# UMich-CURLY/SE3ET

Hardware: AMD Instinct MI355X
Metric: point-cloud pairs/sec (fwd), SE3ET-E 5k-pt pairs (higher is better)
Workload: dtype f32

## Files before the change

### include/se3et_hip.h

```cpp
#ifndef SE3ET_HIP_H_
#define SE3ET_HIP_H_

#include <stddef.h>
#include <stdint.h>

#ifdef __cplusplus
extern "C" {
#endif

#define SE3_OK 0
#define SE3_ERR_INVALID_ARG 1
#define SE3_ERR_UNSUPPORTED 2
#define SE3_ERR_LAUNCH 3
#define SE3_ERR_WORKSPACE 4

#define SE3_MAX_BATCH 32
#define SE3_MAX_NEIGHBOR_LIMIT 64

const char* se3_version(void);
const char* se3_last_error(void);
void se3_debug_set_sinkhorn_variant(int variant);
unsigned long long se3_debug_dense_saturated_rows(int reset);
unsigned long long se3_debug_attention_saturated(int reset);
void se3_debug_kernel_timing(int enable);
// ... 72 lines not shown
                         const float* residual_affine, float final_slope, int64_t rows, int channels,
                         const int64_t* segment_row_offsets_host, int num_segments, int blocked_layout, float* out, void* stream);
int se3_group_norm_apply_amax(const float* x, const float* affine_a, float slope_a, const float* affine_b, float slope_b, const float* residual,
                              const float* residual_affine, float final_slope, int64_t rows, int channels,
                              const int64_t* segment_row_offsets_host, int num_segments, int blocked_layout, float* out, float* amax_out,
                              void* stream);
size_t se3_dense_norm_workspace_bytes(int groups);
int se3_dense_norm_fwd(const float* x, int64_t rows, int in_features, const float* in_affine_a, float in_slope_a, const float* in_affine_b,
                       float in_slope_b, const void* weight_pieces, int out_features, const float* linear_bias, const float* norm_weight,
                       const float* norm_bias, int groups, float eps, const int64_t* segment_row_offsets_host, int num_segments, float* out,
                       float* affine_out, void* workspace, size_t workspace_bytes, void* stream);
int se3_dense_residual_fwd(const float* x, int64_t rows, int in_features, const float* in_affine_a, float in_slope_a, const float* in_affine_b,
                           float in_slope_b, const void* weight_pieces, const float* affine, const float* x2, int in_features2,
                           const void* weight_pieces2, const float* affine2, const float* residual, int out_features, float final_slope,
                           const int64_t* segment_row_offsets_host, int num_segments, float* out, void* stream);
int se3_linear_stream(const float* x, int64_t rows, int in_features, int64_t x_row_stride, const void* weight_pieces, const float* bias,
                      int out_features, int apply_relu, float* out, int64_t out_row_stride, void* stream);
int se3_linear_stream_transposed(const float* x, int64_t rows, int in_features, int64_t x_row_stride, const void* weight_pieces,
                                 const float* bias, int out_features, int block_rows, float* out_t, int64_t ld, void* stream);

int se3_add_layer_norm_fwd(const float* hidden, const float* hidden_bias, const float* residual, const float* weight,
                           const float* bias, int64_t rows, int64_t residual_rows, int channels, float eps, float* out,
                           void* stream);
int se3_add_layer_norm_bwd(const float* hidden, const float* hidden_bias, const float* residual, const float* weight,
                           const float* grad_out, int64_t rows, int64_t residual_rows, int channels, float eps, float* grad_hidden,
                           float* grad_params, void* stream);

size_t se3_linear_weight_pieces_bytes(int out_features, int in_features);
int se3_linear_split_weights_f16(const float* weight, int out_features, int in_features, void* pieces, void* stream);
int se3_linear_f16(const float* x, int64_t rows, int in_features, int64_t x_row_stride, const void* weight_pieces, const float* bias,
                   int out_features, int apply_relu, float* out, int64_t out_row_stride, void* stream);

int se3_gather_rows_padded(const float* x, const int64_t* idx, int64_t n, int64_t m, int64_t width, float* out,
                           void* stream);
int se3_neighbor_max_pool(const float* x, const int64_t* idx, int64_t n, int64_t m, int nn, int64_t width, float* out,
                          void* stream);
int se3_neighbor_max_pool_bwd(const float* x, const int64_t* idx, const float* dout, int64_t n, int64_t m, int nn, int64_t width,
                              float* dx, void* stream);
int se3_anchor_max(const float* x, int num_anchors, int64_t rows, int channels, int64_t anchor_stride, int64_t row_stride,
                   float* out, void* stream);

int se3_kpconv_so3_gather(const float* q_pts, const float* s_pts, const int64_t* idx, const float* x,
                          const float* kernel_points_host, const int64_t* kidx_host, const int64_t* ridx_host, float sigma,
                          int64_t num_queries, int64_t num_support, int num_neighbors, int in_channels, float* G,
                          void* stream);
int se3_kpconv_so3_gather_bwd(const float* q_pts, const float* s_pts, const int64_t* idx, const float* dG,
// ... 544 lines not shown
```

### se3et_amd/csrc/dense_norm.hip

```cpp
#include "common.h"
#include "group_norm.h"

namespace {

using f16x8 = __attribute__((ext_vector_type(8))) _Float16;
using f16x4 = __attribute__((ext_vector_type(4))) _Float16;
using f32x16 = __attribute__((ext_vector_type(16))) float;
using f32x4 = __attribute__((ext_vector_type(4))) float;
using u32x4 = __attribute__((ext_vector_type(4))) unsigned;
using i32x4 = __attribute__((ext_vector_type(4))) int;

__device__ unsigned long long g_dense_saturated_rows = 0;

template <int CTRL>
__device__ __forceinline__ float dpp_f32(float v) {
  return __builtin_bit_cast(float, __builtin_amdgcn_update_dpp(0, __builtin_bit_cast(int, v), CTRL, 0xf, 0xf, true));
}

constexpr int kHeaderB = 256;
constexpr int kRowB = 80;

struct DenseArgs {
  const float* x;
  const float* in_affine[2];
// ... 4 lines not shown
  float* out;
  float* part;
  int* counters;
  const float* xb;
  const float* gw;
  const float* gb;
  float* affine;
  int groups;
  float eps;
  SegTable T;
  const float* affine1;
  const float* residual;
  const float* x2;
  int K2;
  const u32x4* Wf2;
  const float* hdr2;
  const float* affine2;
  float final_slope;
  int x_rs, out_rs;
  int t_rows;
  int t_ld;
  int seg_steps;
  long long seg_stride;
};


struct StepPos {
  int tile, kk;
};
template <int WM, int WN, int RT, int CT, int MODE>
__global__ __launch_bounds__(256, MODE == 3 ? 2 : 3) void dense_norm_kernel(const DenseArgs a) {
  static_assert(WM * WN == 4, "4 waves");
  constexpr int TR = 32 * RT * WM, BN = 32 * CT * WN, U = TR / 32;
  constexpr int kPieceB = TR * kRowB, kBufB = 2 * kPieceB;
  constexpr bool kStats = MODE <= 1, kDual = MODE == 3, kPlain = MODE >= 4;
  __shared__ __align__(16) unsigned char lds[2 * kBufB];
  __shared__ __align__(16) int row_exp[2][TR];
  __shared__ __align__(16) int row_exp_step[2][TR];
  __shared__ int row_run[TR];
  __shared__ int row_scl[2];
  extern __shared__ __align__(16) float aff[];
  const int tid = threadIdx.x, lane = tid & 63, wave = __builtin_amdgcn_readfirstlane(tid >> 6);
  const int wm = wave / WN, wn = wave % WN;
  const int i32 = lane & 31, h = lane >> 5;
  const int K = a.K, N = a.N;
  const int K2 = kDual ? a.K2 : 32;
  const int XS = kPlain ? a.x_rs : K, OS = kPlain ? a.out_rs : N;
  long long r0, r1;
  chunk_rows(a.T, blockIdx.x, r0, r1);
  if (r1 < r0) r1 = r0;
  const int seg = seg_of_chunk(a.T, blockIdx.x);
  int cb0 = a.T.chunk_begin[0], cb1 = a.T.chunk_begin[1];
#pragma unroll
  for (int i = 1; i < kGNMaxSegments; i++)
// ... 151 lines not shown
    }
    const bool w_scaled = __builtin_amdgcn_ballot_w64(any_scaled) != 0;
    plain_rows = !w_scaled;
    if (last_step && w_scaled && lane == 0) row_scl[buf] = p.tile * nkt + p.kk;
    if (saturated) atomicAdd(&g_dense_saturated_rows, (unsigned long long)saturated);
  };
  const int a_read = (wm * (RT * 32) + i32) * kRowB + h * 16;
  const int ct0 = blockIdx.y * (BN / 32) + wn * CT;
  const u32x4* wbase1 = a.Wf + (int64_t)ct0 * 2 * 64 + lane;
  const u32x4* wbase2 = kDual ? a.Wf2 + (int64_t)ct0 * 2 * 64 + lane : wbase1;
  int coff[CT];
#pragma unroll
  for (int c = 0; c < CT; c++) coff[c] = kPlain ? ((ct0 + c < a.NCT ? ct0 + c : a.NCT - 1) - ct0) * 128 : c * 128;
  const int64_t wstep = (int64_t)a.NCT * 2 * 64;
  const float inv_scale = a.hdr[0];
  float fs[CT], bs[CT], rescale[CT];
#pragma unroll
  for (int c = 0; c < CT; c++) fs[c] = bs[c] = rescale[c] = 1.f;
  if constexpr (kPlain) {
#pragma unroll
    for (int c = 0; c < CT; c++) {
      const int col = (ct0 + c) * 32 + i32;
      fs[c] = inv_scale;
      bs[c] = (a.xb != nullptr && col < N) ? a.xb[col] : 0.f;
    }
  } else if constexpr (MODE >= 2) {
#pragma unroll
    for (int c = 0; c < CT; c++) {
      const int col = (ct0 + c) * 32 + i32;
      const float a1 = a.affine1[(size_t)seg * 2 * N + col], b1 = a.affine1[(size_t)seg * 2 * N + N + col];
      if constexpr (kDual) {
        const float a2 = a.affine2[(size_t)seg * 2 * N + col], b2 = a.affine2[(size_t)seg * 2 * N + N + col];
        const float inv2 = a.hdr2[0];
        rescale[c] = (a1 / a2) * (inv_scale / inv2);
        fs[c] = a2 * inv2;
        bs[c] = b1 + b2;
      } else {
        fs[c] = a1 * inv_scale;
        bs[c] = b1;
      }
    }
  }
  f32x16 acc[RT][CT];
#pragma unroll
  for (int r = 0; r < RT; r++)
#pragma unroll
    for (int c = 0; c < CT; c++)
// ... 107 lines not shown
    if constexpr (MODE == 5) {
      const __amdgpu_buffer_rsrc_t ors = __builtin_amdgcn_make_buffer_rsrc(a.out, 0, 0x7ffffff0, 0x00020000);
#pragma unroll
      for (int c = 0; c < CT; c++) {
        const int col = (ct0 + c) * 32 + i32;
#pragma unroll
        for (int r = 0; r < RT; r++)
#pragma unroll
          for (int g = 0; g < 4; g++) {
            const long long row = trow0 + r * 32 + 8 * g + 4 * h;
            const int blk = (int)(row / a.t_rows), rloc = (int)(row - (long long)blk * a.t_rows);
            f32x4 v4;
#pragma unroll
            for (int j = 0; j < 4; j++) {
              float val = acc[r][c][4 * g + j] * fs[c] + bs[c];
              v4[j] = fmaxf(val, val * a.final_slope);
              acc[r][c][4 * g + j] = 0.f;
            }
            const bool ok = col < N && row < r1;
            const int off = ok ? (int)((((long long)blk * N + col) * a.t_ld + rloc) * 4) : 0x7ffffff0;
            __builtin_amdgcn_raw_buffer_store_b128(__builtin_bit_cast(u32x4, v4), ors, off, 0, 0);
          }
      }
      return;
    }
    if constexpr (MODE >= 2) {
      const __amdgpu_buffer_rsrc_t ors = __builtin_amdgcn_make_buffer_rsrc(a.out + trow0 * N, 0, rows_here * N * 4, 0x00020000);
      const bool has_res = MODE == 2 && a.residual != nullptr;
      const __amdgpu_buffer_rsrc_t rrs = __builtin_amdgcn_make_buffer_rsrc(const_cast<float*>(has_res ? a.residual + trow0 * N : a.out), 0,
                                                                           has_res ? rows_here * N * 4 : 0, 0x00020000);
#pragma unroll
      for (int c = 0; c < CT; c++) {
        const int lane_off = (4 * h * N + (ct0 + c) * 32 + i32) * 4;
#pragma unroll
        for (int r = 0; r < RT; r++) {
          float res[16];
          if constexpr (MODE == 2) {
#pragma unroll
            for (int v = 0; v < 16; v++)
              res[v] = __builtin_bit_cast(float, __builtin_amdgcn_raw_buffer_load_b32(rrs, lane_off, (r * 32 + (v & 3) + 8 * (v >> 2)) * N * 4, 0));
          }
#pragma unroll
          for (int v = 0; v < 16; v++) {
            const int rr = r * 32 + (v & 3) + 8 * (v >> 2);
            float val = acc[r][c][v] * fs[c] + bs[c];
            if constexpr (MODE == 2) val += res[v];
// ... 95 lines not shown
#pragma unroll
    for (int c = 0; c < CT; c++) run[c].mean += a.xb[(ct0 + c) * 32 + i32];
  if (h == 0)
#pragma unroll
    for (int c = 0; c < CT; c++) sh[(wave * CT + c) * 32 + i32] = run[c];
  __syncthreads();
  if (wm == 0)
#pragma unroll
    for (int c = 0; c < CT; c++) {
      WF w = run[c];
      for (int m = 1; m < WM; m++) w = wf_merge(w, sh[((m * WN + wn) * CT + c) * 32 + i32]);
      for (int d = 1; d < cpg; d <<= 1) {
        const WF o = {__shfl_xor(w.n, d), __shfl_xor(w.mean, d), __shfl_xor(w.m2, d)};
        w = wf_merge(w, o);
      }
      const int col = (ct0 + c) * 32 + i32;
      if (h == 0 && (col & (cpg - 1)) == 0) gn_store_partial(a.part + ((int64_t)blockIdx.x * a.groups + col / cpg) * 3, w);
    }
  if (!gn_last_arrival(a.counters + seg * kGNMaxColumnBlocks + blockIdx.y, cb1 - cb0)) return;
  const int gpb = BN / cpg;
  gn_finalize_groups(a.part, a.groups, cb0, cb1, blockIdx.y * gpb, gpb, cpg, a.xb, a.gw, a.gb, a.eps, a.affine + (size_t)seg * 2 * N, N);
}

constexpr int kTargetChunks = 768;

}

extern "C" unsigned long long se3_debug_dense_saturated_rows(int reset) {
  unsigned long long n = 0;
  if (hipMemcpyFromSymbol(&n, HIP_SYMBOL(g_dense_saturated_rows), sizeof(n)) != hipSuccess) return ~0ull;
  if (reset) {
    const unsigned long long zero = 0;
    (void)hipMemcpyToSymbol(HIP_SYMBOL(g_dense_saturated_rows), &zero, sizeof(zero));
  }
  return n;
}

constexpr size_t kCounterB = kGNCounterB;

extern "C" size_t se3_dense_norm_workspace_bytes(int groups) {
  return kCounterB + (size_t)(kGNMaxChunks + kGNMaxSegments) * (groups > 0 ? groups : 1) * 3 * sizeof(float);
}

namespace {
int dense_chunks(int64_t rows, int N, const int64_t* segment_row_offsets_host, int num_segments, SegTable& T, int& TR, int& BN, int& ncb,
                 bool given = false) {
  if (!given) {
    TR = N >= 256 ? 64 : 128;
    BN = N >= 256 ? 256 : N;
  }
  ncb = (N + BN - 1) / BN;
  T = SegTable{};
  T.n = num_segments;
  T.quantum = TR;
  int64_t tiles = 0;
  for (int s = 0; s < num_segments; s++) {
    const int64_t b0 = num_segments == 1 ? 0 : segment_row_offsets_host[s], b1 = num_segments == 1 ? rows : segment_row_offsets_host[s + 1];
    if (!(b1 > b0 && b0 >= 0 && b1 <= rows)) return -1;
    tiles += se3_cdiv(b1 - b0, TR);
  }
  int64_t want = kTargetChunks / ncb;
  if (want > kGNMaxChunks - num_segments) want = kGNMaxChunks - num_segments;
  if (want < 1) want = 1;
  int64_t tiles_per_chunk = se3_cdiv(tiles, want);
  for (int s = 0; s < num_segments; s++) {
    const int64_t b0 = num_segments == 1 ? 0 : segment_row_offsets_host[s], b1 = num_segments == 1 ? rows : segment_row_offsets_host[s + 1];
    const int64_t need = se3_cdiv(se3_cdiv(b1 - b0, TR), 256);
    if (need > tiles_per_chunk) tiles_per_chunk = need;
  }
  int chunks = 0;
  for (int s = 0; s < num_segments; s++) {
    const int64_t b0 = num_segments == 1 ? 0 : segment_row_offsets_host[s], b1 = num_segments == 1 ? rows : segment_row_offsets_host[s + 1];
    T.row_begin[s] = b0;
    T.row_begin[s + 1] = b1;
    T.chunk_begin[s] = chunks;
    chunks += (int)se3_cdiv(se3_cdiv(b1 - b0, TR), tiles_per_chunk);
    T.chunk_begin[s + 1] = chunks;
  }
  if (!(T.row_begin[0] == 0 && T.row_begin[num_segments] == rows && chunks <= kGNMaxChunks + kGNMaxSegments)) return -1;
  return chunks;
}

template <int MODE>
void dense_launch(const DenseArgs& a, int N, dim3 grid, size_t dyn, hipStream_t st) {
// ... 99 lines not shown
  hipStream_t st = (hipStream_t)stream;
  const dim3 grid((unsigned)chunks, (unsigned)ncb);
  if (x2 != nullptr) {
    a.x2 = x2;
    a.K2 = K2;
    a.hdr2 = static_cast<const float*>(weight_pieces2);
    a.Wf2 = reinterpret_cast<const u32x4*>(static_cast<const unsigned char*>(weight_pieces2) + kHeaderB);
    a.affine2 = affine2;
    dense_launch<3>(a, N, grid, dyn, st);
  } else {
    dense_launch<2>(a, N, grid, dyn, st);
  }
  SE3_CHECK_LAUNCH("dense_residual");
  return SE3_OK;
}


namespace {
template <int WM, int WN, int RT, int CT>
void plain_launch(const DenseArgs& a, bool transposed, dim3 grid, hipStream_t st) {
  if (transposed) dense_norm_kernel<WM, WN, RT, CT, 5><<<grid, 256, 0, st>>>(a);
  else dense_norm_kernel<WM, WN, RT, CT, 4><<<grid, 256, 0, st>>>(a);
}
int linear_stream_one(const float* x, int64_t rows, int K, int64_t x_rs, const void* weight_pieces, const float* bias, int N, int relu, float* out,
                      int64_t out_rs, int t_rows, int64_t t_ld, void* stream, int seg_channels = 0, int64_t seg_stride = 0) {
  SE3_REQUIRE(x && weight_pieces && out, SE3_ERR_INVALID_ARG, "linear_stream: null pointer");
  SE3_REQUIRE(K > 0 && K % 32 == 0 && N > 0, SE3_ERR_UNSUPPORTED, "linear_stream: in_features %d must be a multiple of 32", K);
  SE3_REQUIRE(x_rs >= 4 && x_rs % 4 == 0 && ((uintptr_t)x & 15) == 0 && rows * x_rs < (1ll << 29), SE3_ERR_INVALID_ARG,
              "linear_stream: x rows must be 16-byte aligned, row stride %lld, below 2 GB", (long long)x_rs);
  const bool transposed = t_rows > 0;
  if (transposed)
    SE3_REQUIRE(t_rows % 4 == 0 && rows % t_rows == 0 && t_ld >= t_rows && t_ld % 4 == 0 && ((uintptr_t)out & 15) == 0 &&
                    (rows / t_rows) * N * t_ld < (1ll << 29),
                SE3_ERR_INVALID_ARG, "linear_stream: transposed output blocks of %d rows (a multiple of 4 dividing %lld), leading dimension %lld",
                t_rows, (long long)rows, (long long)t_ld);
  else
    SE3_REQUIRE(out_rs >= N && rows * out_rs < (1ll << 29), SE3_ERR_INVALID_ARG, "linear_stream: out row stride %lld", (long long)out_rs);
  if (rows == 0) return SE3_OK;
  int TR, BN, cfg;
  const int64_t rt64 = se3_cdiv(rows, 64);
  if (N > 128) {
    if (rt64 * se3_cdiv(N, 256) >= 512) { TR = 64; BN = 256; cfg = 0; }
    else if (rt64 * se3_cdiv(N, 128) >= 320 || N % 128 > 64) { TR = 64; BN = 128; cfg = 1; }
    else { TR = 64; BN = 64; cfg = 2; }
  } else if (N > 64) { TR = rt64 >= 512 ? 128 : 64; BN = 128; cfg = rt64 >= 512 ? 3 : 1; }
  else if (N > 32) { TR = rt64 >= 512 ? 128 : 64; BN = 64; cfg = rt64 >= 512 ? 4 : 2; }
  else { TR = 128; BN = 32; cfg = 5; }
  if (transposed && cfg == 3) { TR = 64; cfg = 1; }
  SegTable T;
  int ncb;
  const int chunks = dense_chunks(rows, N, nullptr, 1, T, TR, BN, ncb, true);
  SE3_REQUIRE(chunks > 0, SE3_ERR_INVALID_ARG, "linear_stream: %lld rows", (long long)rows);
  DenseArgs a{};
  a.x = x;
  a.K = K;
  a.N = N;
  a.NCT = (N + 63) / 64 * 2;
  a.hdr = static_cast<const float*>(weight_pieces);
  a.Wf = reinterpret_cast<const u32x4*>(static_cast<const unsigned char*>(weight_pieces) + kHeaderB);
  a.out = out;
  a.xb = bias;
  a.T = T;
  a.final_slope = relu ? 0.f : 1.f;
  a.x_rs = (int)x_rs;
  a.out_rs = (int)out_rs;
  a.t_rows = t_rows;
  a.t_ld = (int)t_ld;
  if (seg_channels > 0) {
    SE3_REQUIRE(seg_channels % 32 == 0 && K % seg_channels == 0 && seg_stride >= rows * x_rs && (K / seg_channels) * seg_stride < (1ll << 29),
                SE3_ERR_INVALID_ARG, "linear_stream: %d input channels in segments of %d", K, seg_channels);
    a.seg_steps = seg_channels / 32;
    a.seg_stride = seg_stride;
  }
  hipStream_t st = (hipStream_t)stream;
  const dim3 grid((unsigned)chunks, (unsigned)ncb);
  switch (cfg) {
    case 0: plain_launch<1, 4, 2, 2>(a, transposed, grid, st); break;
    case 1: plain_launch<2, 2, 1, 2>(a, transposed, grid, st); break;
    case 2: plain_launch<2, 2, 1, 1>(a, transposed, grid, st); break;
    case 3: plain_launch<2, 2, 2, 2>(a, transposed, grid, st); break;
    case 4: plain_launch<4, 1, 1, 2>(a, transposed, grid, st); break;
    default: plain_launch<4, 1, 1, 1>(a, transposed, grid, st); break;
  }
  SE3_CHECK_LAUNCH("linear_stream");
  return SE3_OK;
}

int linear_stream(const float* x, int64_t rows, int K, int64_t x_rs, const void* weight_pieces, const float* bias, int N, int relu, float* out,
                  int64_t out_rs, int t_rows, int64_t t_ld, void* stream, int seg_channels = 0, int64_t seg_stride = 0) {
  const int64_t lim = (1ll << 29) - 1;
  const bool transposed = t_rows > 0;
  const bool fits = rows >= 0 && x_rs > 0 && rows * x_rs <= lim &&
                    (transposed ? (rows / t_rows) * (int64_t)N * t_ld <= lim : rows * (out_rs > N ? out_rs : (int64_t)N) <= lim);
  if (fits || seg_channels > 0 || !x || !out || N <= 0) return linear_stream_one(x, rows, K, x_rs, weight_pieces, bias, N, relu, out, out_rs, t_rows, t_ld, stream, seg_channels, seg_stride);
  int64_t step;
  if (transposed) {
    SE3_REQUIRE(rows % t_rows == 0 && t_ld >= t_rows, SE3_ERR_INVALID_ARG, "linear_stream: transposed output blocks of %d rows", t_rows);
    const int64_t per_block = std::max((int64_t)t_rows * x_rs, (int64_t)N * t_ld);
    SE3_REQUIRE(per_block <= lim, SE3_ERR_UNSUPPORTED, "linear_stream: one transposed block of %d rows exceeds 2 GB", t_rows);
    step = lim / per_block * t_rows;
  } else {
    SE3_REQUIRE(out_rs >= N, SE3_ERR_INVALID_ARG, "linear_stream: out row stride %lld", (long long)out_rs);
    step = lim / std::max(x_rs, out_rs) / 256 * 256;
    SE3_REQUIRE(step > 0, SE3_ERR_UNSUPPORTED, "linear_stream: row strides %lld / %lld too large", (long long)x_rs, (long long)out_rs);
  }
  for (int64_t r0 = 0; r0 < rows; r0 += step) {
    const int64_t n = std::min(step, rows - r0);
    float* o = transposed ? out + (r0 / t_rows) * (int64_t)N * t_ld : out + r0 * out_rs;
    const int rc = linear_stream_one(x + r0 * x_rs, n, K, x_rs, weight_pieces, bias, N, relu, o, out_rs, t_rows, t_ld, stream);
    if (rc != SE3_OK) return rc;
  }
  return SE3_OK;
}
}

extern "C" int se3_linear_stream(const float* x, int64_t rows, int in_features, int64_t x_row_stride, const void* weight_pieces, const float* bias,
                                 int out_features, int apply_relu, float* out, int64_t out_row_stride, void* stream) {
  return linear_stream(x, rows, in_features, x_row_stride, weight_pieces, bias, out_features, apply_relu, out, out_row_stride, 0, 0, stream);
}

extern "C" int se3_linear_stream_transposed(const float* x, int64_t rows, int in_features, int64_t x_row_stride, const void* weight_pieces,
                                            const float* bias, int out_features, int block_rows, float* out_t, int64_t ld, void* stream) {
  SE3_REQUIRE(block_rows > 0, SE3_ERR_INVALID_ARG, "linear_stream_transposed: block_rows %d", block_rows);
  return linear_stream(x, rows, in_features, x_row_stride, weight_pieces, bias, out_features, 0, out_t, 0, block_rows, ld, stream);
}


extern "C" int se3_linear_stream_segments(const float* x, int64_t rows, int in_features, int seg_channels, int64_t seg_stride,
                                          const void* weight_pieces, const float* bias, int out_features, int apply_relu, float* out,
                                          int64_t out_row_stride, void* stream) {
  SE3_REQUIRE(seg_channels > 0, SE3_ERR_INVALID_ARG, "linear_stream_segments: seg_channels %d", seg_channels);
  return linear_stream(x, rows, in_features, seg_channels, weight_pieces, bias, out_features, apply_relu, out, out_row_stride, 0, 0, stream,
                       seg_channels, seg_stride);
}
```

### se3et_amd/csrc/transformer_driver.hip

```cpp
#include <cstddef>
#include <hip/hip_runtime.h>

#include <cmath>
#include <cstring>

#include "../../include/se3et_hip.h"
#include "common.h"

namespace {

struct Arena {
  unsigned char* base;
  size_t size, used;
  bool ok;
  void* take(size_t bytes) {
    const size_t at = se3_align256(used);
    if (at + bytes > size) {
      ok = false;
      return base;
    }
    used = at + bytes;
    return base + at;
  }
  float* floats(size_t n) { return static_cast<float*>(take(n * sizeof(float))); }
};

struct Half {
  int64_t row0, rows;
  int64_t starts[SE3_MAX_BATCH], lengths[SE3_MAX_BATCH];
  int n;
};

#define SE3_TRY(call)          \
  do {                         \
    const int rc_ = (call);    \
    if (rc_ != SE3_OK) return rc_; \
  } while (0)

int dense(const se3_linear_t& L, const float* x, int64_t rows, float* out, int relu, bool with_bias, void* st) {
  return se3_linear_stream(x, rows, L.in_features, L.in_features, L.pieces, with_bias ? L.bias : nullptr, L.out_features, relu, out,
                           L.out_features, st);
}

int ffn(const se3_layer_t& L, const float* y, int64_t rows, int C, float* out, Arena& S, void* st) {
  float* mid = S.floats((size_t)rows * L.expand.out_features);
  float* sq = S.floats((size_t)rows * C);
  if (!S.ok) return SE3_ERR_WORKSPACE;
  SE3_TRY(dense(L.expand, y, rows, mid, 1, true, st));
  SE3_TRY(dense(L.squeeze, mid, rows, sq, 0, false, st));
  return se3_add_layer_norm_fwd(sq, L.squeeze.bias, y, L.ln2_w, L.ln2_b, rows, rows, C, L.ln2_eps, out, st);
}

int copy_rows(float* dst, int64_t dst_pitch_floats, const float* src, int64_t src_pitch_floats, int64_t width_floats, int64_t height, hipStream_t st) {
  if (hipMemcpy2DAsync(dst, (size_t)dst_pitch_floats * 4, src, (size_t)src_pitch_floats * 4, (size_t)width_floats * 4, (size_t)height,
                       hipMemcpyDeviceToDevice, st) != hipSuccess) {
    se3_set_error("transformer_forward: device copy failed");
    return SE3_ERR_LAUNCH;
  }
  return SE3_OK;
}

int zero(float* p, size_t n, hipStream_t st) {
  if (hipMemsetAsync(p, 0, n * sizeof(float), st) != hipSuccess) {
    se3_set_error("transformer_forward: memset failed");
    return SE3_ERR_LAUNCH;
  }
  return SE3_OK;
}

int eq_groups(int A, const Half& q, int H, int C, const Half& k, int64_t v_row_stride) {
  if (C / H != 64 || C % H || A > 6 || v_row_stride % 16) return 1;
  for (int i = 0; i < k.n; i++)
    if (k.starts[i] % 16) return 1;
// ... 85 lines not shown
      float* vt = W.floats((size_t)As * C * R);
      float* hidden = W.floats((size_t)rows * C);
      size_t lg = 0;
      for (int c = 0; c < 2 * B; c++) lg += (size_t)As * H * plan->lengths[c] * ((plan->lengths[c] + 31) / 32 * 32);
      float* logits = W.floats(lg);
      const size_t kvb = se3_attention_kv_pieces_bytes(As, R, C, (int)R);
      void* kv = kvb ? W.take(kvb) : nullptr;
      float* lin = W.floats((size_t)rows * C);
      float* y = W.floats((size_t)rows * C);
      if (!W.ok) { se3_set_error("transformer_forward: workspace exhausted (self block %d)", bi); return SE3_ERR_WORKSPACE; }
      SE3_TRY(dense(L.stack, src, rows, proj, 0, true, stream));
      SE3_TRY(se3_linear_stream_transposed(src, rows, C, C, L.v.pieces, L.v.bias, C, (int)R, vt, R, stream));
      SE3_TRY(zero(hidden, (size_t)rows * C, st));
      const float* const* eqp = eq ? plan->eq : nullptr;
      const float* qe = eq ? proj + L.off_qe : nullptr;
      if (plan->emb_bf16)
        SE3_TRY(se3_rpe_self_attention_stack_bf16_fwd(proj + L.off_q, proj + L.off_k, vt, proj + L.off_qp, qe, NS, As > 1 ? (int64_t)R * NS : 0, (int)R,
                                                      As > 1 ? (int64_t)C * R : 0, reinterpret_cast<const uint16_t* const*>(plan->emb), eqp, plan->starts,
                                                      plan->lengths, 2 * B, As, C, H, logits, As > 1 ? (int64_t)R * C : 0, hidden, kv, kvb, stream));
      else
        SE3_TRY(se3_rpe_self_attention_stack_fwd(proj + L.off_q, proj + L.off_k, vt, proj + L.off_qp, qe, NS, As > 1 ? (int64_t)R * NS : 0, (int)R,
                                                 As > 1 ? (int64_t)C * R : 0, plan->emb, eqp, plan->starts, plan->lengths, 2 * B, As, C, H, logits,
                                                 As > 1 ? (int64_t)R * C : 0, hidden, kv, kvb, stream));
      SE3_TRY(dense(L.out, hidden, rows, lin, 0, false, stream));
      SE3_TRY(se3_add_layer_norm_fwd(lin, L.out.bias, src, L.ln1_w, L.ln1_b, rows, rows, C, L.ln1_eps, y, stream));
      float* Xn = free_slot(X, Xeq);
      SE3_TRY(ffn(L, y, rows, C, Xn, W, stream));
      if (L.type == 1 && next == 2) {
        float* inv = free_slot(Xn, X, Xeq);
        SE3_TRY(se3_anchor_max(Xn, A, R, C, (int64_t)R * C, C, inv, stream));
        Xeq = Xn;
        X = inv;
        X_is_eq = false;
      } else {
        X = Xn;
        X_is_eq = As > 1;
      }
    } else if (L.type == 2) {
      SE3_REQUIRE(!X_is_eq, SE3_ERR_UNSUPPORTED, "transformer_forward: block %d: plain cross attention on anchor features", bi);
      const bool eq_values = next == 1 || (next < 0 && prev == 1);
      SE3_REQUIRE(!eq_values || Xeq != nullptr, SE3_ERR_INVALID_ARG, "transformer_forward: block %d needs the anchor features of a self_eq block", bi);
      const int Av = eq_values ? A : 1;
      float* Xn = free_slot(X, Xeq);
      float* Xeqn = eq_values ? free_slot(X, Xeq, Xn) : nullptr;
      auto direction = [&](const Half& Pq, const Half& Pk, const float* xq, const float* xk, const float* xv, int64_t xv_pitch, float* y_out ) -> int {
        const int64_t Rq = Pq.rows, Rk = Pk.rows;
        float* q = W.floats((size_t)Rq * C);
        float* k = W.floats((size_t)Rk * C);
        float* xvc = W.floats((size_t)Av * Rk * C);
        float* vt = W.floats((size_t)Av * C * Rk);
        float* hidden = W.floats((size_t)Av * Rq * C);
        float* lin = W.floats((size_t)Av * Rq * C);
        float* y = W.floats((size_t)Av * Rq * C);
        if (!W.ok) { se3_set_error("transformer_forward: workspace exhausted (cross block %d)", bi); return SE3_ERR_WORKSPACE; }
        SE3_TRY(dense(L.q, xq, Rq, q, 0, true, stream));
        SE3_TRY(dense(L.k, xk, Rk, k, 0, true, stream));
        const float* xvv = xv;
        if (Av > 1 && xv_pitch != Rk * C) {
          SE3_TRY(copy_rows(xvc, Rk * C, xv, xv_pitch, Rk * C, Av, st));
          xvv = xvc;
        }
        SE3_TRY(se3_linear_stream_transposed(xvv, (int64_t)Av * Rk, C, C, L.v.pieces, L.v.bias, C, (int)Rk, vt, Rk, stream));
        SE3_TRY(zero(hidden, (size_t)Av * Rq * C, st));
        SE3_TRY(se3_attention_stack_fwd(q, k, vt, nullptr, Pq.starts, Pq.lengths, Pk.starts, Pk.lengths, nullptr, Pq.n, Av, C, H, C, C, (int)Rk, 0, 0,
                                        Av > 1 ? (int64_t)C * Rk : 0, Av > 1 ? (int64_t)Rq * C : 0, scale, hidden, nullptr, 0, stream));
        SE3_TRY(dense(L.out, hidden, (int64_t)Av * Rq, lin, 0, false, stream));
        SE3_TRY(se3_add_layer_norm_fwd(lin, L.out.bias, xq, L.ln1_w, L.ln1_b, (int64_t)Av * Rq, Rq, C, L.ln1_eps, y, stream));
        return ffn(L, y, (int64_t)Av * Rq, C, y_out, W, stream);
      };
      if (eq_values) {
        float* y0 = W.floats((size_t)A * R0 * C);
        float* y1 = W.floats((size_t)A * R1 * C);
        SE3_TRY(direction(P0, P1, X, X + R0 * C, Xeq + R0 * C, (int64_t)R * C, y0));
        SE3_TRY(se3_anchor_max(y0, A, R0, C, (int64_t)R0 * C, C, Xn, stream));
        SE3_TRY(direction(P1, P0, X + R0 * C, Xn, y0, (int64_t)R0 * C, y1));
        SE3_TRY(se3_anchor_max(y1, A, R1, C, (int64_t)R1 * C, C, Xn + R0 * C, stream));
        SE3_TRY(copy_rows(Xeqn, R * C, y0, R0 * C, R0 * C, A, st));
        SE3_TRY(copy_rows(Xeqn + R0 * C, R * C, y1, R1 * C, R1 * C, A, st));
        Xeq = Xeqn;
      } else {
        SE3_TRY(direction(P0, P1, X, X + R0 * C, X + R0 * C, 0, Xn));
        SE3_TRY(direction(P1, P0, X + R0 * C, Xn, Xn, 0, Xn + R0 * C));
      }
      X = Xn;
      X_is_eq = false;
    } else {
      SE3_REQUIRE(X_is_eq && A == 6, SE3_ERR_UNSUPPORTED, "transformer_forward: block %d: equivariant cross attention needs (6, rows, C) features", bi);
      const int mode = L.type == 3 ? 0 : 1;
      float* y0 = W.floats((size_t)A * R0 * C);
      float* y1 = W.floats((size_t)A * R1 * C);
// ... 8 lines not shown
        float* hidden = W.floats((size_t)A * Rq * G * C);
        float* gq = W.floats((size_t)A * B * C * C);
        float* gk = W.floats((size_t)A * B * C * C);
        float* partial = W.floats((size_t)B * A * A);
        float* weights = W.floats((size_t)B * (mode == 0 ? A * A : L.num_rotations));
        const size_t x6b = se3_cross_eq_x6_workspace_bytes(A, Rq, Rk, C, (int)Rk);
        void* x6 = W.take(x6b);
        float* lin = W.floats((size_t)A * Rq * C);
        float* y = W.floats((size_t)A * Rq * C);
        if (!W.ok) { se3_set_error("transformer_forward: workspace exhausted (equivariant cross block %d)", bi); return SE3_ERR_WORKSPACE; }
        SE3_TRY(dense(L.q, xq, (int64_t)A * Rq, q, 0, true, stream));
        SE3_TRY(dense(L.k, xk, (int64_t)A * Rk, k, 0, true, stream));
        SE3_TRY(se3_linear_stream_transposed(xk, (int64_t)A * Rk, C, C, L.v.pieces, L.v.bias, C, (int)Rk, vt, Rk, stream));
        SE3_TRY(zero(hidden, (size_t)A * Rq * G * C, st));
        SE3_TRY(se3_gram_stack(q, A, C, (int64_t)Rq * C, Pq.starts, Pq.lengths, B, gq, stream));
        SE3_TRY(se3_gram_stack(k, A, C, (int64_t)Rk * C, Pk.starts, Pk.lengths, B, gk, stream));
        const float f = 1.0f / (std::sqrt((float)(C / H)) * (float)H);
        SE3_TRY(se3_gram_frobenius(gq, gk, A, B, (int64_t)C * C, f * f, partial, stream));
        SE3_TRY(se3_cross_eq_stack_x6_fwd(q, k, vt, Pq.starts, Pq.lengths, Pk.starts, Pk.lengths, B, A, C, H, Rq, Rk, (int64_t)Rq * C, (int64_t)Rk * C,
                                          (int)Rk, (int64_t)C * Rk, mode, L.trace_idx, L.num_rotations, 1, partial, mix, weights, hidden, G,
                                          (int64_t)Rq * G * C, x6, x6b, stream));
        const void* wp = G == 1 ? L.out.pieces : (G == 2 ? L.out_pieces_g2 : L.out_pieces_g3);
        SE3_REQUIRE(wp != nullptr, SE3_ERR_INVALID_ARG, "transformer_forward: block %d: no output projection for %d key-anchor groups", bi, G);
        SE3_TRY(se3_linear_stream(hidden, (int64_t)A * Rq, G * C, (int64_t)G * C, wp, nullptr, C, 0, lin, C, stream));
        SE3_TRY(se3_add_layer_norm_fwd(lin, L.out.bias, xq, L.ln1_w, L.ln1_b, (int64_t)A * Rq, (int64_t)A * Rq, C, L.ln1_eps, y, stream));
        return ffn(L, y, (int64_t)A * Rq, C, y_out, W, stream);
      };
      float* xq0 = W.floats((size_t)A * R0 * C);
      float* xk0 = W.floats((size_t)A * R1 * C);
      if (!W.ok) { se3_set_error("transformer_forward: workspace exhausted (equivariant cross block %d)", bi); return SE3_ERR_WORKSPACE; }
      SE3_TRY(copy_rows(xq0, R0 * C, X, R * C, R0 * C, A, st));
      SE3_TRY(copy_rows(xk0, R1 * C, X + R0 * C, R * C, R1 * C, A, st));
      SE3_TRY(direction(P0, P1, xq0, xk0, mix0, y0));
      SE3_TRY(direction(P1, P0, xk0, y0, mix1, y1));
      float* Xn = free_slot(X, Xeq);
      if (L.type == 4 && next >= 0 && next != 1 && next < 3) {
        SE3_REQUIRE(plan->rc_expand.pieces && plan->rc_squeeze.pieces, SE3_ERR_INVALID_ARG, "transformer_forward: block %d needs the rotcompress layer", bi);
        float* y1p = W.floats((size_t)A * R1 * C);
        SE3_TRY(se3_anchor_mix_stack(y1, R1, C, mix0, P1.starts, P1.lengths, B, y1p, stream));
        auto rotcompress = [&](const float* x, int64_t Rh, float* o) -> int {
          float* mx = W.floats((size_t)Rh * C);
          float* mid = W.floats((size_t)Rh * plan->rc_expand.out_features);
          float* sq = W.floats((size_t)Rh * C);
          if (!W.ok) { se3_set_error("transformer_forward: workspace exhausted (rotcompress)"); return SE3_ERR_WORKSPACE; }
          SE3_TRY(se3_anchor_max(x, A, Rh, C, Rh * C, C, mx, stream));
          SE3_TRY(se3_linear_stream_segments(x, Rh, A * C, C, Rh * C, plan->rc_expand.pieces, plan->rc_expand.bias, plan->rc_expand.out_features, 1, mid,
                                             plan->rc_expand.out_features, stream));
          SE3_TRY(dense(plan->rc_squeeze, mid, Rh, sq, 0, false, stream));
          return se3_add_layer_norm_fwd(sq, plan->rc_squeeze.bias, mx, plan->rc_ln_w, plan->rc_ln_b, Rh, Rh, C, plan->rc_ln_eps, o, stream);
        };
        SE3_TRY(rotcompress(y0, R0, Xn));
        SE3_TRY(rotcompress(y1p, R1, Xn + R0 * C));
        X = Xn;
        X_is_eq = false;
        Xeq = nullptr;
      } else {
        SE3_TRY(copy_rows(Xn, R * C, y0, R0 * C, R0 * C, A, st));
        SE3_TRY(copy_rows(Xn + R0 * C, R * C, y1, R1 * C, R1 * C, A, st));
        X = Xn;
        X_is_eq = true;
      }
    }
  }
  SE3_REQUIRE(!X_is_eq, SE3_ERR_UNSUPPORTED, "transformer_forward: the block list must end on invariant features");
  return dense(plan->out_proj, X, R, out, 0, true, stream);
}
```

### se3et_amd/ops.py

```python
import ctypes
import os
import threading

import torch

from .caches import CACHE_EPOCH, Derived, Workspace, _Shared, also_clear, clear_caches, clear_weight_caches, validate_weight_caches
from ._lib import CONSTANTS, ENUMS, check, lib
from .stacking import PAIR_MAX_PAIRS, device_offsets, exclusive_offsets, to_device


_HAS_BLAS_SWITCH = hasattr(torch.backends.cuda, 'preferred_blas_library')
if _HAS_BLAS_SWITCH:
    torch.backends.cuda.preferred_blas_library('cublas')
_BLAS_SWITCH_LOCK = threading.Lock()
_BIG_GEMM_FLOP = 2.0e9


def mm(a, b):
    big = 2.0 * a.shape[0] * a.shape[1] * b.shape[1] > _BIG_GEMM_FLOP
    if _HAS_BLAS_SWITCH and big and (b.stride(-1) == 1 or a.shape[1] <= 32):
        with _BLAS_SWITCH_LOCK:
            torch.backends.cuda.preferred_blas_library('cublaslt')
            try:
                return torch.mm(a, b)
# ... 85 lines not shown
    if out is None:
        out = torch.empty(x.shape[:-1] + (N,), dtype=torch.float32, device=x.device)
        out_rs = N
    else:
        if out.dim() != 2 or out.shape[0] != rows or out.shape[1] != N or out.stride(1) != 1 or out.dtype != torch.float32:
            raise RuntimeError('linear_stream: out must be a (rows, N) float32 view with unit column stride')
        out_rs = out.stride(0)
    b = None if bias is None else _req(bias.detach().contiguous(), torch.float32, 'bias', 1)
    check(lib().se3_linear_stream(x.data_ptr(), rows, K, x_rs, Wp.data_ptr(), None if b is None else b.data_ptr(), N, 1 if relu else 0,
                                  out.data_ptr(), out_rs, stream), 'se3_linear_stream')
    return out


def linear_stream_transposed(x, weight, bias, ld=None):
    A, R, K = x.shape
    N = weight.shape[0]
    ld = R if ld is None else int(ld)
    stream = _stream()
    Wp = _linear_weight_pieces(weight, stream)
    out = torch.empty((A, N, ld), dtype=torch.float32, device=x.device)
    b = None if bias is None else _req(bias.detach().contiguous(), torch.float32, 'bias', 1)
    check(lib().se3_linear_stream_transposed(x.data_ptr(), A * R, K, K, Wp.data_ptr(), None if b is None else b.data_ptr(), N, R, out.data_ptr(), ld,
                                             stream), 'se3_linear_stream_transposed')
    return out


TIMING_TAG = None
KERNEL_TIMINGS = None
_TIMING_LOCK = threading.Lock()


class _timed:
    def __init__(self, name, nbytes, kind=None):
        self.name, self.nbytes, self.kind = name, nbytes, kind

    def __enter__(self):
        if KERNEL_TIMINGS is not None:
            self.e0, self.e1 = torch.cuda.Event(enable_timing=True), torch.cuda.Event(enable_timing=True)
            self.e0.record()

    def __exit__(self, *exc):
        if KERNEL_TIMINGS is not None:
            self.e1.record()
            KERNEL_TIMINGS.setdefault(self.name, []).append((self.e0, self.e1, self.nbytes))
            if self.kind is not None:
                KERNEL_TIMINGS.setdefault(self.name + '/' + self.kind, []).append((self.e0, self.e1, self.nbytes))
# ... 2477 lines not shown
```

Baseline: 465.5.

## Fuse output projection with residual add and LayerNorm in linear stream kernel

Adds a new epilogue mode to the dense GEMM kernel that adds bias and residual, computes per-row mean and variance through a cross-wave LDS reduction, and writes LayerNorm output directly. The transformer driver's attention-output, FFN-squeeze and rotation-compress projections now use this fused path instead of a GEMM followed by a separate add-layernorm launch. This removes one kernel launch and a full write/read round-trip of the intermediate per call. In exchange, each block must cover the full row width (128 or 256 columns), which constrains tiling and occupancy and adds two block syncs.

Measured after the change: 461.1. No clear change (-0.9%).

```diff
diff --git a/include/se3et_hip.h b/include/se3et_hip.h
--- a/include/se3et_hip.h
+++ b/include/se3et_hip.h
@@ -118,6 +118,9 @@
 int se3_add_layer_norm_fwd(const float* hidden, const float* hidden_bias, const float* residual, const float* weight,
                            const float* bias, int64_t rows, int64_t residual_rows, int channels, float eps, float* out,
                            void* stream);
+int se3_linear_layer_norm_stream(const float* x, int64_t rows, int in_features, int64_t x_row_stride, const void* weight_pieces,
+                                 const float* linear_bias, int out_features, const float* residual, int64_t residual_rows,
+                                 const float* ln_weight, const float* ln_bias, float eps, float* out, float* scratch, void* stream);
 int se3_add_layer_norm_bwd(const float* hidden, const float* hidden_bias, const float* residual, const float* weight,
                            const float* grad_out, int64_t rows, int64_t residual_rows, int channels, float eps, float* grad_hidden,
                            float* grad_params, void* stream);
diff --git a/se3et_amd/csrc/dense_norm.hip b/se3et_amd/csrc/dense_norm.hip
--- a/se3et_amd/csrc/dense_norm.hip
+++ b/se3et_amd/csrc/dense_norm.hip
@@ -50,6 +50,12 @@
   int t_ld;
   int seg_steps;
   long long seg_stride;
+  const float* ln_w;
+  const float* ln_b;
+  float ln_eps;
+  int res_rows;
+  int res_row0;
+  int res_bytes;
 };
 
 
@@ -57,7 +63,7 @@
   int tile, kk;
 };
 template <int WM, int WN, int RT, int CT, int MODE>
-__global__ __launch_bounds__(256, MODE == 3 ? 2 : 3) void dense_norm_kernel(const DenseArgs a) {
+__global__ __launch_bounds__(256, (MODE == 3 || (MODE == 6 && (RT == 2 || WM == 2))) ? 2 : 3) void dense_norm_kernel(const DenseArgs a) {
   static_assert(WM * WN == 4, "4 waves");
   constexpr int TR = 32 * RT * WM, BN = 32 * CT * WN, U = TR / 32;
   constexpr int kPieceB = TR * kRowB, kBufB = 2 * kPieceB;
@@ -255,7 +261,7 @@
     for (int c = 0; c < CT; c++) {
       const int col = (ct0 + c) * 32 + i32;
       fs[c] = inv_scale;
-      bs[c] = (a.xb != nullptr && col < N) ? a.xb[col] : 0.f;
+      bs[c] = (MODE != 6 && a.xb != nullptr && col < N) ? a.xb[col] : 0.f;
     }
   } else if constexpr (MODE >= 2) {
 #pragma unroll
@@ -409,6 +415,127 @@
             __builtin_amdgcn_raw_buffer_store_b128(__builtin_bit_cast(u32x4, v4), ors, off, 0, 0);
           }
       }
+      return;
+    }
+    if constexpr (MODE == 6) {
+#pragma clang fp contract(off)
+      int tid_here = tid;
+      asm volatile("" : "+v"(tid_here));
+      const int lane = tid_here & 63, i32 = lane & 31, h = lane >> 5;
+      static_assert(MODE != 6 || (CT == 2 && (WN == 2 || WN == 4)), "LayerNorm epilogue: two column tiles per wave, 2 or 4 column waves");
+      constexpr int NP = 8 * WN * CT, kLd = NP + 8;
+      __shared__ __align__(16) float ln_part[TR][kLd];
+      __shared__ __align__(16) float ln_tot[2][TR];
+      constexpr float inv_n = 1.0f / BN;
+      auto put = [&](int r, int g, int c, f32x4 t) {
+#pragma unroll
+        for (int j = 0; j < 4; j++) {
+          t[j] += dpp_f32<0xB1>(t[j]);
+          t[j] += dpp_f32<0x4E>(t[j]);
+        }
+        const int j = i32 & 3;
+        const float mine = j == 0 ? t[0] : (j == 1 ? t[1] : (j == 2 ? t[2] : t[3]));
+        ln_part[(wm * RT + r) * 32 + 8 * g + 4 * h + j][(wn * CT + c) * 8 + (i32 >> 2)] = mine;
+      };
+      auto reduce = [&](int pass) {
+#pragma unroll
+        for (int it = 0; it < TR / 32; it++) {
+          const int row = (it * 4 + wave) * 8 + (lane >> 3), j = lane & 7;
+          float pk[WN * CT];
+#pragma unroll
+          for (int k = 0; k < WN * CT; k++) pk[k] = ln_part[row][k * 8 + j];
+          if (pass == 0) {
+#pragma unroll
+            for (int k = 0; k < WN * CT; k++) pk[k] = 0.f + pk[k];
+          }
+          float t;
+          if constexpr (WN == 4) t = ((pk[0] + pk[4]) + (pk[2] + pk[6])) + ((pk[1] + pk[5]) + (pk[3] + pk[7]));
+          else t = (pk[0] + pk[2]) + (pk[1] + pk[3]);
+          t += __shfl_xor(t, 4);
+          t += dpp_f32<0x4E>(t);
+          t += dpp_f32<0xB1>(t);
+          t = t * inv_n;
+          if (pass == 1) t = 1.0f / sqrtf(t + a.ln_eps);
+          if (j == 0) ln_tot[pass][row] = t;
+        }
+      };
+      const __amdgpu_buffer_rsrc_t rrs = __builtin_amdgcn_make_buffer_rsrc(const_cast<float*>(a.residual), 0, a.res_bytes, 0x00020000);
+      const __amdgpu_buffer_rsrc_t ors = __builtin_amdgcn_make_buffer_rsrc(a.out + trow0 * OS, 0, rows_here > 0 ? ((rows_here - 1) * OS + N) * 4 : 0, 0x00020000);
+      const int grow0 = (int)trow0 + 4 * h;
+      const bool bcast = a.res_rows > 0;
+      float bias[CT];
+#pragma unroll
+      for (int c = 0; c < CT; c++) bias[c] = a.xb != nullptr ? a.xb[(ct0 + c) * 32 + i32] : 0.f;
+      float res[RT][CT][16];
+#pragma unroll
+      for (int r = 0; r < RT; r++)
+#pragma unroll
+        for (int v = 0; v < 16; v++) {
+          const int row = grow0 + r * 32 + (v & 3) + 8 * (v >> 2);
+          const int roff = (bcast ? (int)((unsigned)(row + a.res_row0) % (unsigned)a.res_rows) : row) * N * 4;
+#pragma unroll
+          for (int c = 0; c < CT; c++)
+            res[r][c][v] = __builtin_bit_cast(float, __builtin_amdgcn_raw_buffer_load_b32(rrs, roff + ((ct0 + c) * 32 + i32) * 4, 0, 0));
+        }
+#pragma unroll
+      for (int r = 0; r < RT; r++)
+#pragma unroll
+        for (int g = 0; g < 4; g++)
+#pragma unroll
+          for (int c = 0; c < CT; c++) {
+            f32x4 t;
+#pragma unroll
+            for (int j = 0; j < 4; j++) {
+              const float val = (acc[r][c][4 * g + j] * fs[c] + bias[c]) + res[r][c][4 * g + j];
+              acc[r][c][4 * g + j] = val;
+              t[j] = val;
+            }
+            put(r, g, c, t);
+          }
+      __syncthreads();
+      reduce(0);
+      __syncthreads();
+#pragma unroll
+      for (int r = 0; r < RT; r++)
+#pragma unroll
+        for (int g = 0; g < 4; g++) {
+          const f32x4 mean = *reinterpret_cast<const f32x4*>(&ln_tot[0][(wm * RT + r) * 32 + 8 * g + 4 * h]);
+#pragma unroll
+          for (int c = 0; c < CT; c++) {
+            f32x4 t;
+#pragma unroll
+            for (int j = 0; j < 4; j++) {
+              const float d = acc[r][c][4 * g + j] - mean[j];
+              acc[r][c][4 * g + j] = d;
+              t[j] = d * d;
+            }
+            put(r, g, c, t);
+          }
+        }
+      __syncthreads();
+      reduce(1);
+      __syncthreads();
+      float lw[CT], lb[CT];
+#pragma unroll
+      for (int c = 0; c < CT; c++) {
+        lw[c] = a.ln_w[(ct0 + c) * 32 + i32];
+        lb[c] = a.ln_b[(ct0 + c) * 32 + i32];
+      }
+#pragma unroll
+      for (int r = 0; r < RT; r++)
+#pragma unroll
+        for (int g = 0; g < 4; g++) {
+          const f32x4 rstd = *reinterpret_cast<const f32x4*>(&ln_tot[1][(wm * RT + r) * 32 + 8 * g + 4 * h]);
+#pragma unroll
+          for (int j = 0; j < 4; j++)
+#pragma unroll
+            for (int c = 0; c < CT; c++) {
+              const float val = __builtin_fmaf(acc[r][c][4 * g + j] * rstd[j], lw[c], lb[c]);
+              __builtin_amdgcn_raw_buffer_store_b32(__builtin_bit_cast(unsigned, val), ors, (4 * h * OS + (ct0 + c) * 32 + i32) * 4,
+                                                    (r * 32 + 8 * g + j) * OS * 4, 0);
+              acc[r][c][4 * g + j] = 0.f;
+            }
+        }
       return;
     }
     if constexpr (MODE >= 2) {
@@ -550,6 +677,7 @@
   gn_finalize_groups(a.part, a.groups, cb0, cb1, blockIdx.y * gpb, gpb, cpg, a.xb, a.gw, a.gb, a.eps, a.affine + (size_t)seg * 2 * N, N);
 }
 
+constexpr int kLnSmallTileRows = 8192;
 constexpr int kTargetChunks = 768;
 
 }
@@ -572,7 +700,7 @@
 
 namespace {
 int dense_chunks(int64_t rows, int N, const int64_t* segment_row_offsets_host, int num_segments, SegTable& T, int& TR, int& BN, int& ncb,
-                 bool given = false) {
+                 bool given = false, int target = kTargetChunks) {
   if (!given) {
     TR = N >= 256 ? 64 : 128;
     BN = N >= 256 ? 256 : N;
@@ -587,7 +715,7 @@
     if (!(b1 > b0 && b0 >= 0 && b1 <= rows)) return -1;
     tiles += se3_cdiv(b1 - b0, TR);
   }
-  int64_t want = kTargetChunks / ncb;
+  int64_t want = target / ncb;
   if (want > kGNMaxChunks - num_segments) want = kGNMaxChunks - num_segments;
   if (want < 1) want = 1;
   int64_t tiles_per_chunk = se3_cdiv(tiles, want);
@@ -733,8 +861,18 @@
   if (transposed) dense_norm_kernel<WM, WN, RT, CT, 5><<<grid, 256, 0, st>>>(a);
   else dense_norm_kernel<WM, WN, RT, CT, 4><<<grid, 256, 0, st>>>(a);
 }
+struct LnTail {
+  const float* residual;
+  int64_t res_rows, row0;
+  const float* w;
+  const float* b;
+  float eps;
+};
+bool ln_tail_covers(int N, int64_t out_rs, int64_t res_rows) { return (N == 128 || N == 256) && out_rs == N && res_rows * N < (1ll << 29); }
+
 int linear_stream_one(const float* x, int64_t rows, int K, int64_t x_rs, const void* weight_pieces, const float* bias, int N, int relu, float* out,
-                      int64_t out_rs, int t_rows, int64_t t_ld, void* stream, int seg_channels = 0, int64_t seg_stride = 0) {
+                      int64_t out_rs, int t_rows, int64_t t_ld, void* stream, int seg_channels = 0, int64_t seg_stride = 0,
+                      const LnTail* ln = nullptr) {
   SE3_REQUIRE(x && weight_pieces && out, SE3_ERR_INVALID_ARG, "linear_stream: null pointer");
   SE3_REQUIRE(K > 0 && K % 32 == 0 && N > 0, SE3_ERR_UNSUPPORTED, "linear_stream: in_features %d must be a multiple of 32", K);
   SE3_REQUIRE(x_rs >= 4 && x_rs % 4 == 0 && ((uintptr_t)x & 15) == 0 && rows * x_rs < (1ll << 29), SE3_ERR_INVALID_ARG,
@@ -758,9 +896,16 @@
   else if (N > 32) { TR = rt64 >= 512 ? 128 : 64; BN = 64; cfg = rt64 >= 512 ? 4 : 2; }
   else { TR = 128; BN = 32; cfg = 5; }
   if (transposed && cfg == 3) { TR = 64; cfg = 1; }
+  if (ln != nullptr) {
+    SE3_REQUIRE(!transposed && !relu && ln->residual && ln->w && ln->b && ln_tail_covers(N, out_rs, ln->res_rows), SE3_ERR_UNSUPPORTED,
+                "linear_layer_norm: %d output features, row stride %lld", N, (long long)out_rs);
+    BN = N;
+    if (N == 256) { TR = rt64 >= kLnSmallTileRows / 64 ? 64 : 32; cfg = TR == 64 ? 6 : 7; }
+    else { TR = 64; cfg = 8; }
+  }
   SegTable T;
   int ncb;
-  const int chunks = dense_chunks(rows, N, nullptr, 1, T, TR, BN, ncb, true);
+  const int chunks = dense_chunks(rows, N, nullptr, 1, T, TR, BN, ncb, true, (cfg == 6 || cfg == 8) ? 512 : kTargetChunks);
   SE3_REQUIRE(chunks > 0, SE3_ERR_INVALID_ARG, "linear_stream: %lld rows", (long long)rows);
   DenseArgs a{};
   a.x = x;
@@ -783,6 +928,15 @@
     a.seg_steps = seg_channels / 32;
     a.seg_stride = seg_stride;
   }
+  if (ln != nullptr) {
+    a.residual = ln->residual;
+    a.ln_w = ln->w;
+    a.ln_b = ln->b;
+    a.ln_eps = ln->eps;
+    a.res_rows = (int)ln->res_rows;
+    a.res_row0 = (int)ln->row0;
+    a.res_bytes = (int)((ln->res_rows > 0 ? ln->res_rows : rows) * N * 4);
+  }
   hipStream_t st = (hipStream_t)stream;
   const dim3 grid((unsigned)chunks, (unsigned)ncb);
   switch (cfg) {
@@ -791,6 +945,9 @@
     case 2: plain_launch<2, 2, 1, 1>(a, transposed, grid, st); break;
     case 3: plain_launch<2, 2, 2, 2>(a, transposed, grid, st); break;
     case 4: plain_launch<4, 1, 1, 2>(a, transposed, grid, st); break;
+    case 6: dense_norm_kernel<1, 4, 2, 2, 6><<<grid, 256, 0, st>>>(a); break;
+    case 7: dense_norm_kernel<1, 4, 1, 2, 6><<<grid, 256, 0, st>>>(a); break;
+    case 8: dense_norm_kernel<2, 2, 1, 2, 6><<<grid, 256, 0, st>>>(a); break;
     default: plain_launch<4, 1, 1, 1>(a, transposed, grid, st); break;
   }
   SE3_CHECK_LAUNCH("linear_stream");
@@ -798,12 +955,12 @@
 }
 
 int linear_stream(const float* x, int64_t rows, int K, int64_t x_rs, const void* weight_pieces, const float* bias, int N, int relu, float* out,
-                  int64_t out_rs, int t_rows, int64_t t_ld, void* stream, int seg_channels = 0, int64_t seg_stride = 0) {
+                  int64_t out_rs, int t_rows, int64_t t_ld, void* stream, int seg_channels = 0, int64_t seg_stride = 0, const LnTail* ln = nullptr) {
   const int64_t lim = (1ll << 29) - 1;
   const bool transposed = t_rows > 0;
   const bool fits = rows >= 0 && x_rs > 0 && rows * x_rs <= lim &&
                     (transposed ? (rows / t_rows) * (int64_t)N * t_ld <= lim : rows * (out_rs > N ? out_rs : (int64_t)N) <= lim);
-  if (fits || seg_channels > 0 || !x || !out || N <= 0) return linear_stream_one(x, rows, K, x_rs, weight_pieces, bias, N, relu, out, out_rs, t_rows, t_ld, stream, seg_channels, seg_stride);
+  if (fits || seg_channels > 0 || !x || !out || N <= 0) return linear_stream_one(x, rows, K, x_rs, weight_pieces, bias, N, relu, out, out_rs, t_rows, t_ld, stream, seg_channels, seg_stride, ln);
   int64_t step;
   if (transposed) {
     SE3_REQUIRE(rows % t_rows == 0 && t_ld >= t_rows, SE3_ERR_INVALID_ARG, "linear_stream: transposed output blocks of %d rows", t_rows);
@@ -818,7 +975,13 @@
   for (int64_t r0 = 0; r0 < rows; r0 += step) {
     const int64_t n = std::min(step, rows - r0);
     float* o = transposed ? out + (r0 / t_rows) * (int64_t)N * t_ld : out + r0 * out_rs;
-    const int rc = linear_stream_one(x + r0 * x_rs, n, K, x_rs, weight_pieces, bias, N, relu, o, out_rs, t_rows, t_ld, stream);
+    LnTail part{};
+    if (ln != nullptr) {
+      part = *ln;
+      if (ln->res_rows > 0) part.row0 = (ln->row0 + r0) % ln->res_rows;
+      else part.residual = ln->residual + r0 * N;
+    }
+    const int rc = linear_stream_one(x + r0 * x_rs, n, K, x_rs, weight_pieces, bias, N, relu, o, out_rs, t_rows, t_ld, stream, 0, 0, ln ? &part : nullptr);
     if (rc != SE3_OK) return rc;
   }
   return SE3_OK;
@@ -828,6 +991,23 @@
 extern "C" int se3_linear_stream(const float* x, int64_t rows, int in_features, int64_t x_row_stride, const void* weight_pieces, const float* bias,
                                  int out_features, int apply_relu, float* out, int64_t out_row_stride, void* stream) {
   return linear_stream(x, rows, in_features, x_row_stride, weight_pieces, bias, out_features, apply_relu, out, out_row_stride, 0, 0, stream);
+}
+
+extern "C" int se3_linear_layer_norm_stream(const float* x, int64_t rows, int in_features, int64_t x_row_stride, const void* weight_pieces,
+                                            const float* linear_bias, int out_features, const float* residual, int64_t residual_rows,
+                                            const float* ln_weight, const float* ln_bias, float eps, float* out, float* scratch, void* stream) {
+  SE3_REQUIRE(x && weight_pieces && residual && ln_weight && ln_bias && out, SE3_ERR_INVALID_ARG, "linear_layer_norm: null pointer");
+  SE3_REQUIRE(rows >= 0 && residual_rows >= 1 && rows % residual_rows == 0, SE3_ERR_INVALID_ARG,
+              "linear_layer_norm: rows %lld not a multiple of residual rows %lld", (long long)rows, (long long)residual_rows);
+  const int N = out_features;
+  if (!ln_tail_covers(N, N, residual_rows == rows ? 0 : residual_rows)) {
+    SE3_REQUIRE(scratch != nullptr, SE3_ERR_WORKSPACE, "linear_layer_norm: %d output features need the scratch buffer of the two-launch path", N);
+    const int rc = linear_stream(x, rows, in_features, x_row_stride, weight_pieces, nullptr, N, 0, scratch, N, 0, 0, stream);
+    if (rc != SE3_OK) return rc;
+    return se3_add_layer_norm_fwd(scratch, linear_bias, residual, ln_weight, ln_bias, rows, residual_rows, N, eps, out, stream);
+  }
+  const LnTail ln{residual, residual_rows == rows ? 0 : residual_rows, 0, ln_weight, ln_bias, eps};
+  return linear_stream(x, rows, in_features, x_row_stride, weight_pieces, linear_bias, N, 0, out, N, 0, 0, stream, 0, 0, &ln);
 }
 
 extern "C" int se3_linear_stream_transposed(const float* x, int64_t rows, int in_features, int64_t x_row_stride, const void* weight_pieces,
diff --git a/se3et_amd/csrc/transformer_driver.hip b/se3et_amd/csrc/transformer_driver.hip
--- a/se3et_amd/csrc/transformer_driver.hip
+++ b/se3et_amd/csrc/transformer_driver.hip
@@ -42,13 +42,18 @@
                            L.out_features, st);
 }
 
+int dense_ln(const se3_linear_t& L, const float* x, int64_t rows, const float* residual, int64_t res_rows, const float* ln_w, const float* ln_b,
+             float eps, float* out, float* lin, void* st) {
+  return se3_linear_layer_norm_stream(x, rows, L.in_features, L.in_features, L.pieces, L.bias, L.out_features, residual, res_rows, ln_w, ln_b,
+                                      eps, out, lin, st);
+}
+
 int ffn(const se3_layer_t& L, const float* y, int64_t rows, int C, float* out, Arena& S, void* st) {
   float* mid = S.floats((size_t)rows * L.expand.out_features);
   float* sq = S.floats((size_t)rows * C);
   if (!S.ok) return SE3_ERR_WORKSPACE;
   SE3_TRY(dense(L.expand, y, rows, mid, 1, true, st));
-  SE3_TRY(dense(L.squeeze, mid, rows, sq, 0, false, st));
-  return se3_add_layer_norm_fwd(sq, L.squeeze.bias, y, L.ln2_w, L.ln2_b, rows, rows, C, L.ln2_eps, out, st);
+  return dense_ln(L.squeeze, mid, rows, y, rows, L.ln2_w, L.ln2_b, L.ln2_eps, out, sq, st);
 }
 
 int copy_rows(float* dst, int64_t dst_pitch_floats, const float* src, int64_t src_pitch_floats, int64_t width_floats, int64_t height, hipStream_t st) {
@@ -180,8 +185,7 @@
         SE3_TRY(se3_rpe_self_attention_stack_fwd(proj + L.off_q, proj + L.off_k, vt, proj + L.off_qp, qe, NS, As > 1 ? (int64_t)R * NS : 0, (int)R,
                                                  As > 1 ? (int64_t)C * R : 0, plan->emb, eqp, plan->starts, plan->lengths, 2 * B, As, C, H, logits,
                                                  As > 1 ? (int64_t)R * C : 0, hidden, kv, kvb, stream));
-      SE3_TRY(dense(L.out, hidden, rows, lin, 0, false, stream));
-      SE3_TRY(se3_add_layer_norm_fwd(lin, L.out.bias, src, L.ln1_w, L.ln1_b, rows, rows, C, L.ln1_eps, y, stream));
+      SE3_TRY(dense_ln(L.out, hidden, rows, src, rows, L.ln1_w, L.ln1_b, L.ln1_eps, y, lin, stream));
       float* Xn = free_slot(X, Xeq);
       SE3_TRY(ffn(L, y, rows, C, Xn, W, stream));
       if (L.type == 1 && next == 2) {
@@ -222,8 +226,7 @@
         SE3_TRY(zero(hidden, (size_t)Av * Rq * C, st));
         SE3_TRY(se3_attention_stack_fwd(q, k, vt, nullptr, Pq.starts, Pq.lengths, Pk.starts, Pk.lengths, nullptr, Pq.n, Av, C, H, C, C, (int)Rk, 0, 0,
                                         Av > 1 ? (int64_t)C * Rk : 0, Av > 1 ? (int64_t)Rq * C : 0, scale, hidden, nullptr, 0, stream));
-        SE3_TRY(dense(L.out, hidden, (int64_t)Av * Rq, lin, 0, false, stream));
-        SE3_TRY(se3_add_layer_norm_fwd(lin, L.out.bias, xq, L.ln1_w, L.ln1_b, (int64_t)Av * Rq, Rq, C, L.ln1_eps, y, stream));
+        SE3_TRY(dense_ln(L.out, hidden, (int64_t)Av * Rq, xq, Rq, L.ln1_w, L.ln1_b, L.ln1_eps, y, lin, stream));
         return ffn(L, y, (int64_t)Av * Rq, C, y_out, W, stream);
       };
       if (eq_values) {
@@ -278,8 +281,8 @@
                                           (int64_t)Rq * G * C, x6, x6b, stream));
         const void* wp = G == 1 ? L.out.pieces : (G == 2 ? L.out_pieces_g2 : L.out_pieces_g3);
         SE3_REQUIRE(wp != nullptr, SE3_ERR_INVALID_ARG, "transformer_forward: block %d: no output projection for %d key-anchor groups", bi, G);
-        SE3_TRY(se3_linear_stream(hidden, (int64_t)A * Rq, G * C, (int64_t)G * C, wp, nullptr, C, 0, lin, C, stream));
-        SE3_TRY(se3_add_layer_norm_fwd(lin, L.out.bias, xq, L.ln1_w, L.ln1_b, (int64_t)A * Rq, (int64_t)A * Rq, C, L.ln1_eps, y, stream));
+        SE3_TRY(se3_linear_layer_norm_stream(hidden, (int64_t)A * Rq, G * C, (int64_t)G * C, wp, L.out.bias, C, xq, (int64_t)A * Rq, L.ln1_w, L.ln1_b,
+                                             L.ln1_eps, y, lin, stream));
         return ffn(L, y, (int64_t)A * Rq, C, y_out, W, stream);
       };
       float* xq0 = W.floats((size_t)A * R0 * C);
@@ -302,8 +305,7 @@
           SE3_TRY(se3_anchor_max(x, A, Rh, C, Rh * C, C, mx, stream));
           SE3_TRY(se3_linear_stream_segments(x, Rh, A * C, C, Rh * C, plan->rc_expand.pieces, plan->rc_expand.bias, plan->rc_expand.out_features, 1, mid,
                                              plan->rc_expand.out_features, stream));
-          SE3_TRY(dense(plan->rc_squeeze, mid, Rh, sq, 0, false, stream));
-          return se3_add_layer_norm_fwd(sq, plan->rc_squeeze.bias, mx, plan->rc_ln_w, plan->rc_ln_b, Rh, Rh, C, plan->rc_ln_eps, o, stream);
+          return dense_ln(plan->rc_squeeze, mid, Rh, mx, Rh, plan->rc_ln_w, plan->rc_ln_b, plan->rc_ln_eps, o, sq, stream);
         };
         SE3_TRY(rotcompress(y0, R0, Xn));
         SE3_TRY(rotcompress(y1p, R1, Xn + R0 * C));
diff --git a/se3et_amd/ops.py b/se3et_amd/ops.py
--- a/se3et_amd/ops.py
+++ b/se3et_amd/ops.py
@@ -131,6 +131,23 @@
     b = None if bias is None else _req(bias.detach().contiguous(), torch.float32, 'bias', 1)
     check(lib().se3_linear_stream_transposed(x.data_ptr(), A * R, K, K, Wp.data_ptr(), None if b is None else b.data_ptr(), N, R, out.data_ptr(), ld,
                                              stream), 'se3_linear_stream_transposed')
+    return out
+
+
+def linear_layer_norm_stream(x, weight, bias, residual, ln_weight, ln_bias, eps):
+    stream = _stream()
+    N, K = weight.shape
+    x = _req(x.contiguous(), torch.float32, 'x', 2)
+    residual = _req(residual.contiguous(), torch.float32, 'residual', 2)
+    rows, res_rows = x.shape[0], residual.shape[0]
+    Wp = _linear_weight_pieces(weight, stream)
+    b = None if bias is None else _req(bias.detach().contiguous(), torch.float32, 'bias', 1)
+    lw, lb = _req(ln_weight.detach().contiguous(), torch.float32, 'ln_weight', 1), _req(ln_bias.detach().contiguous(), torch.float32, 'ln_bias', 1)
+    out = torch.empty((rows, N), dtype=torch.float32, device=x.device)
+    scratch = torch.empty((rows, N), dtype=torch.float32, device=x.device)
+    check(lib().se3_linear_layer_norm_stream(x.data_ptr(), rows, K, K, Wp.data_ptr(), None if b is None else b.data_ptr(), N, residual.data_ptr(),
+                                             res_rows, lw.data_ptr(), lb.data_ptr(), float(eps), out.data_ptr(), scratch.data_ptr(), stream),
+          'se3_linear_layer_norm_stream')
     return out
 
 
```
